# rlvc/FEALESS

Measured on AMD Instinct MI355X. Metric: frames/sec (640x480 RGB-D x N templates, 20 ICP iters), higher is better.
Workload: dtype u8

## Files before the change

### fealess_amd/csrc/fl_context.hip

```cpp
#include "fl_internal.h"
#include <stdlib.h>
#include <stdarg.h>
#include <string.h>
#include <algorithm>

int fl_set_error(fl_context *ctx, int code, const char *fmt, ...)
{
  if (ctx) {
    va_list ap;
    va_start(ap, fmt);
    vsnprintf(ctx->err, sizeof(ctx->err), fmt, ap);
    va_end(ap);
  }
  return code;
}

int fl_scratch(fl_context *ctx, size_t bytes, void **out)
{
  if (int rc = fl_context_join(ctx)) return rc;
  if (bytes > ctx->scratch_bytes) {
    if (ctx->scratch) {
      FL_HIP(ctx, hipStreamSynchronize(ctx->stream));
      FL_HIP(ctx, hipFree(ctx->scratch));
      ctx->scratch = nullptr;
// ... 59 lines not shown
  *out = ctx->icp_stream;
  return FL_OK;
}

extern "C" int fl_abi_version(void) { return FL_ABI_VERSION; }

struct FlOptionName { const char *name, *env; long fl_context::Options::*field; bool hex; long lo, hi; };
static const FlOptionName fl_option_names[] = {
  {"scan_prune", "FL_SCAN_PRUNE", &fl_context::Options::scan_prune, false, 0, 1},
  {"scan_prune_mid", "FL_SCAN_PRUNE_MID", &fl_context::Options::scan_prune_mid, true, -1, 0xFF},
  {"scan_prune_lanes", "FL_SCAN_PRUNE_LANES", &fl_context::Options::scan_prune_lanes, false, 0, 1},
  {"scan_prune_step", "FL_SCAN_PRUNE_STEP", &fl_context::Options::scan_prune_step, false, 0, 8},
  {"scan_first", "FL_SCAN_FIRST", &fl_context::Options::scan_first, false, 0, 16},
  {"icp_wide", "FL_ICP_WIDE", &fl_context::Options::icp_wide, false, -1, 1},
  {"icp_occ", "FL_ICP_OCC", &fl_context::Options::icp_occ, false, 0, 5},
  {"icp_order", "FL_ICP_ORDER", &fl_context::Options::icp_order, false, 0, 1},
  {"icp_wg_per_cu", "FL_ICP_WG_PER_CU", &fl_context::Options::icp_wg_per_cu, false, 0, 3},
  {"eager_frontend", "FL_EAGER_FRONTEND", &fl_context::Options::eager_frontend, false, 0, 1},
  {"dev_poison", "FL_DEV_POISON", &fl_context::Options::dev_poison, false, 0, 1},
  {"ws_pad", "FL_DEV_WS_PAD", &fl_context::Options::ws_pad, false, 0, 16l << 20},
  {"pipeline_icp", "FL_PIPELINE_ICP", &fl_context::Options::pipeline_icp, false, 0, 3},
  {"frontend_chunk_rows", "FL_FRONTEND_CHUNK_ROWS", &fl_context::Options::frontend_chunk_rows, false, 0, 60 * 1024},
  {"scan_run", "FL_SCAN_RUN", &fl_context::Options::scan_run, false, 0, 64},
  {"refine_lds", "FL_REFINE_LDS", &fl_context::Options::refine_lds, false, 0, 2},
  {"refine_lds_bytes", "FL_REFINE_LDS_BYTES", &fl_context::Options::refine_lds_bytes, false, 0, FL_REFINE_LDS_BYTES},
  {"verify_fused", "FL_VERIFY_FUSED", &fl_context::Options::verify_fused, false, 0, 1},
  {"verify_fused_px", "FL_VERIFY_FUSED_PX", &fl_context::Options::verify_fused_px, false, 0, FL_VERIFY_FUSED_PX},
};

static bool fl_option_valid(const FlOptionName &o, long v)
// ... 636 lines not shown
```

### fealess_amd/csrc/fl_icp.hip

```cpp
#include "fl_internal.h"
#include <float.h>
#include <math.h>
#include <string.h>
#include <type_traits>
#include <mutex>
#include <map>
#include <utility>

#define ICP_BS_SMALL 256
#define ICP_BS_WIDE 1024
#define ICP_DT 512
#ifdef FL_ICP_PHASES
#define TSTAMP(k) do { if (threadIdx.x == 0) { long long now_ = clock64(); S.tacc[k] += now_ - S.tlast; S.tlast = now_; } } while (0)
#define CH_STAMP_BEGIN long long c_add = 0, c_bar = 0, c_last = clock64()
#define CH_STAMP(v) { const long long now_ = clock64(); v += now_ - c_last; c_last = now_; }
#define CH_STAMP_END(k) { if (threadIdx.x == 0) { S.hist[k] += (unsigned)(c_add >> 4); S.hist[(k) + 1] += (unsigned)(c_bar >> 4); } }
#define PR_STAMP_BARRIER(k, every) { const long long b0_ = clock64(); tile_barrier(); if (threadIdx.x == 64) S.hist[k] += (unsigned)(((clock64() - b0_) * (every)) >> 4); }
#define ST_STAMP_BEGIN long long st_acc[6] = {0, 0, 0, 0, 0, 0}, st_last = clock64()
#define ST_STAMP(k) { const long long now_ = clock64(); st_acc[k] += now_ - st_last; st_last = now_; }
#define ST_ARRIVED(a, b) asm volatile("" :: "v"(a), "v"(b));
#define ST_STAMP_END { if ((threadIdx.x & 63) == 0) for (int k = 0; k < 5; ++k) atomicAdd(&S.stime[k], (unsigned long long)st_acc[k]); }
#else
#define TSTAMP(k) do { } while (0)
#define CH_STAMP_BEGIN
// ... 409 lines not shown
      const float v[8] = {c0.x, c0.y, c0.z, c0.w, c1.x, c1.y, c1.z, c1.w};
#pragma unroll
      for (int k = 0; k < 8; ++k) blk_term(bs, (k < 4 ? 4 * lane + k : 256 + 4 * lane + k - 4) < cnt ? v[k] : 0.0f, isum, bad);
      if (blk_finish(bs, isum, bad, acc)) continue;
    }
    float *dst = buf[b & 1];
    *(float4 *)(dst + 4 * lane) = c0;
    *(float4 *)(dst + 256 + 4 * lane) = c1;
    wave_lds_handover();
    if (lane == 0) acc = chain_tile<NBUF>(dst, cnt, acc);
    acc = uniform_f(acc);
  }
  return acc;
}

template <int MODE, bool DEFER, class SH>
__device__ __forceinline__ float l2dist_phase(SH &S, float *mod, const float *ref, bnd_t *bnd, float *dterm, int n, float thr,
                                             const float *Ropt, const float *Topt)
{
  constexpr bool parity = MODE == FL_ICP_PARITY && !DEFER;
  constexpr int TQ = parity ? SH::TQ : SH::BS;
  const int slot = parity ? S.producer_slot() : (int)threadIdx.x;
  const int clane = parity ? S.chain_lane() : -1;
  int counter = 0, inl = 0;
  double dsum[1] = {0.0};
  float acc = 0.0f;
  const int ntiles = (n + TQ - 1) / TQ;
  constexpr int KB = parity && !SH::BSUM ? ICP_BMACRO : 1;
  static_assert(KB == 1 || sizeof(S.prod) >= (size_t)2 * KB * TQ * sizeof(float), "two blocks of KB tiles of terms fit the A2 tiles");
  auto dbuf = [&](int t) -> float * {
    if (KB == 1) return S.dtile[t & 1];
    const int m = (t + KB - 1) / KB, first = m == 0 ? 0 : (m - 1) * KB + 1;
    return (float *)&S.prod[0][0][0] + ((m & 1) * KB + (t - first)) * TQ;
  };
  struct Row { F3 a, b; float bnd; };
  auto row_load = [&](Row &w, int t) {
    const int i = min(t * TQ + slot, n - 1);
    w.a = ld3_u32(mod, i);
    w.b = ld3_u32(ref, i);
    w.bnd = Ropt ? bnd_ld(bnd, i) : 0.0f;
  };
  auto row_process = [&](const Row &w, int t) {
    const int i = t * TQ + slot;
    float term = 0.0f;
    float a[3] = {w.a.x, w.a.y, w.a.z};
    const float b0 = w.b.x, b1 = w.b.y, b2 = w.b.z;
    if (i < n) {
      if (Ropt) {
        float move = 0.0f;
        if (vvalid(a[2])) {
          float o[3];
          mat_vec(Ropt, a, o);
          o[0] += Topt[0];
          o[1] += Topt[1];
          o[2] += Topt[2];
          const float mx = o[0] - a[0], my = o[1] - a[1], mz = o[2] - a[2];
          move = sqrt_upper(mx * mx + my * my + mz * mz);
          a[0] = o[0];
          a[1] = o[1];
          a[2] = o[2];
          mod[3 * i] = a[0];
// ... 163 lines not shown
__device__ __forceinline__ void pose_accumulate(SH &S)
{
  float RT[3];
  mat_vec(S.Ropt, S.T, RT);
  for (int k = 0; k < 3; ++k) S.T[k] = RT[k] + S.Topt[k];
  mat_mat(S.Ropt, S.R, S.R);
}
__device__ __forceinline__ void icp_result_none(fl_icp_result *res)
{
  for (int i = 0; i < 9; ++i) res->R[i] = 0.f;
  for (int i = 0; i < 3; ++i) res->T[i] = 0.f;
  res->dist_mean = -1.0f; res->px_ratio = 0.f;
  res->iters = 0; res->n_corr_last = 0;
}

template <int MODE, bool ORG, class SH>
__device__ __forceinline__ void icp_run(SH &S, uint8_t *wsb, const IcpWsLayout &L, int n_ref, int n_model,
                        int it_thr, float dmt, float ddt, fl_icp_result *res, const OrgGeom &og)
{
  constexpr int BS = SH::BS, NW = SH::NW;
  float *ref = (float *)(wsb + L.ref), *mod = (float *)(wsb + L.mod);
  float4 *sref = (float4 *)(wsb + L.sref);
  const float *jsrc = ORG ? (const float *)sref : ref;
  const int *idximg = ORG ? (const int *)((const uint8_t *)sref + org_idximg_offset(og.cw * og.ch)) : nullptr;
  int *nn = (int *)(wsb + L.nn);
  bnd_t *bnd = (bnd_t *)(wsb + L.bnd);
  float *nd = (float *)(wsb + L.nd), *dterm = (float *)(wsb + L.dterm);
  const int *perm = (const int *)(wsb + L.perm);
  const float *nrm = (const float *)(wsb + L.nrm);
  int *cell_start = (int *)(wsb + L.cell_start), *cell_cur = (int *)(wsb + L.cell_cur);
  constexpr bool plane = MODE == FL_ICP_POINT_TO_PLANE;
  constexpr int NSUM = plane ? 27 : 15;

  if (threadIdx.x == 0) {
    for (int i = 0; i < 9; ++i) S.R[i] = 0.f;
    for (int i = 0; i < 3; ++i) S.T[i] = 0.f;
    S.iter = 0;
    S.n_corr = 0;
    S.px = 0.f;
#ifdef FL_ICP_PHASES
    for (int i = 0; i < 16; ++i) S.tacc[i] = 0;
    for (int i = 0; i < 40; ++i) S.hist[i] = 0;
    for (int i = 0; i < 8; ++i) S.stime[i] = 0;
// ... 5 lines not shown
  if (n_model < 3 || n_ref < 3 || n_ref < n_model) {
    if (threadIdx.x == 0) icp_result_none(res);
    __syncthreads();
    return;
  }
  if (!ORG) build_grid(S, ref, n_ref, sref, cell_start, cell_cur, L.ncell_max);
  TSTAMP(0);
  for (int i = threadIdx.x; i < n_model; i += BS)
    if (!vvalid(mod[3 * i + 2])) { mod[3 * i] = 0.f; mod[3 * i + 1] = 0.f; mod[3 * i + 2] = 0.f; }
  if (threadIdx.x == 0) {
    S.R[0] = S.R[4] = S.R[8] = 1.f;
    S.dist_diff = FLT_MAX;
  }
  __syncthreads();
  constexpr bool SPEC = BS >= ICP_BS_WIDE && MODE == FL_ICP_PARITY && ORG;
  float mean_ub = l2dist_phase<MODE, SPEC>(S, mod, ref, bnd, dterm, n_model, FLT_MAX, nullptr, nullptr);
  int pending = SPEC ? 1 : 0;
  bool have_nn = false;
  float old_mean = 0.0f;

  const OrgSearchCtx ctx = org_search_ctx(mod, bnd, perm, (const float *)sref, (const float *)(wsb + L.zimg), n_model, og);
  auto chain_and_search = [&](const int pend, const bool want, const float r_lim, const float old_mean_) {
    if (pend && threadIdx.x < 64) {
      const float acc = chain_deferred<SH::CHAIN_NBUF>(dterm, S.dchain, n_model);
      if (threadIdx.x == 0) {
        const int counter = S.cnt, inl = S.inl;
        float dm = acc;
        if (counter > 0) dm /= (float)inl;
        const float new_mean = counter > 0 ? dm : FLT_MAX;
        S.px = counter > 0 ? (float)inl / (float)counter : 0.0f;
        if (pend == 2) {
          S.dist_diff = old_mean_ - new_mean;
          pose_accumulate(S);
        }
        S.dist_mean = new_mean;
        const bool go = (new_mean > dmt) && (S.dist_diff > ddt) && (S.iter < it_thr);
        *(volatile int *)&S.stop = go ? 0 : 1;
      }
    }
    if (want)
      org_search<SH, SPEC>(S, ctx, r_lim, true, [&](bool active, int i, float, float, float, int j, float d) {
        if (active) {
          nn[i] = j;
          nd[i] = d;
          if (j >= 0) bnd_st(bnd, i, sqrt_upper(d));
        }
      });
  };

  for (;;) {
    if (SPEC) {
      const int it_done = __builtin_amdgcn_readfirstlane(S.iter);
      const bool want = !have_nn && it_done >= 1 && it_done < it_thr;
      if (pending || want) {
        const float r_lim = pending ? sqrtf(3.0f * mean_ub) * 1.00001f : sqrtf(3 * S.dist_mean);
        if (threadIdx.x == 0) { S.a1_next = 0; S.stop = 0; }
        __syncthreads();
        chain_and_search(pending, want, uniform_f(r_lim), old_mean);
// ... 33 lines not shown
      } else if (!parity) {
        const float m[3] = {m0, m1, m2}, r[3] = {r0, r1, r2};
#pragma unroll
        for (int a = 0; a < 3; ++a)
#pragma unroll
          for (int b = 0; b < 3; ++b) ds[a * 3 + b] += (double)m[a] * (double)r[b];
#pragma unroll
        for (int q = 0; q < 3; ++q) { ds[9 + q] += (double)m[q]; ds[12 + q] += (double)r[q]; }
      }
    };
    if (!index_pairs && !SPEC) {
      const float r_thr = uniform_f(sqrtf(thr));
      auto on_found = [&](bool active, int i, float qx, float qy, float qz, int j, float d) {
        const bool keep = d <= thr;
        if (active) {
          nn[i] = keep ? j : -1;
          if (j >= 0) bnd_st(bnd, i, sqrt_upper(d));
        }
        if (keep) {
          ++kept;
          if (!parity) { const F3 rv = ld3_u32(jsrc, j); pair_sums(qx, qy, qz, rv.x, rv.y, rv.z, j); }
        }
      };
      if (ORG) {
        if (MODE == FL_ICP_PARITY && NW < 8) org_search_pipe(S, ctx, r_thr, on_found);
        else org_search<SH, SPEC>(S, ctx, r_thr, false, on_found);
      } else {
        const NnGrid G = nn_grid(S);
        int i = threadIdx.x;
        float qx = 0.f, qy = 0.f, qz = 0.f, qb = 0.f;
        if (i < n_model) { const F3 q3 = ld3_u32(mod, i); qx = q3.x; qy = q3.y; qz = q3.z; qb = bnd_ld(bnd, i); }
// ... 24 lines not shown
        bool in;
        F3 m, r;
      };
      constexpr bool ZIMG = ORG && NW < 8;
      const float *zimg = (const float *)(wsb + L.zimg);
      const float inv_cw = uniform_f(1.0f / (float)max(og.cw, 1));
      auto row_load = [&](Row &w, int t) {
        const int i = t * TQ + slot;
        w.in = i < rows;
        const int ic = min(i, rows - 1);
        w.j = ld_u32(nn, ic);
        w.d = SPEC ? ld_u32(nd, ic) : 0.0f;
        w.m = ld3_u32(mod, ic);
      };
      auto row_gather = [&](Row &w) {
        if (!(w.in && (!SPEC || w.d <= thr))) w.j = -1;
        if (ZIMG) w.r.x = ld_u32(zimg, max(w.j, 0));
        else w.r = ld3_u32(jsrc, max(w.j, 0));
      };
      auto row_write = [&](const Row &w, int t) {
        const bool have = w.j >= 0;
        if (SPEC && have) ++kept;
        float (*tile)[SH::TS] = S.prod[t & 1];
        F3 rp = w.r;
        if (ZIMG) {
          const int jj = max(w.j, 0);
          int vv, uu;
          if (ctx.small_crop) {
            vv = (int)(((float)jj + 0.5f) * inv_cw);
            uu = jj - __mul24(vv, og.cw);
            if (uu < 0) { --vv; uu += og.cw; } else if (uu >= og.cw) { ++vv; uu -= og.cw; }
// ... 47 lines not shown
    } else
    for (int t = 0; t < ntiles; ++t) {
      if (slot >= 0) {
        const int i = t * TQ + slot;
        float m[3] = {0.f, 0.f, 0.f}, r[3] = {0.f, 0.f, 0.f};
        bool have_m = false, have_pair = false;
        if (i < rows) {
          if (iter == 1) {
            if (i < n_model) {
              have_m = true;
              have_pair = true;
              if (vvalid(mod[3 * i + 2])) { m[0] = mod[3 * i]; m[1] = mod[3 * i + 1]; m[2] = mod[3 * i + 2]; }
            }
            if (vvalid(ref[3 * i + 2])) { r[0] = ref[3 * i]; r[1] = ref[3 * i + 1]; r[2] = ref[3 * i + 2]; }
          } else {
            const int j = nn[i];
            if (j >= 0) {
              have_m = have_pair = true;
              m[0] = mod[3 * i]; m[1] = mod[3 * i + 1]; m[2] = mod[3 * i + 2];
              r[0] = jsrc[3 * j]; r[1] = jsrc[3 * j + 1]; r[2] = jsrc[3 * j + 2];
            }
          }
        }
        if (parity) {
          float (*tile)[SH::TS] = S.prod[t & 1];
#pragma unroll
          for (int a = 0; a < 3; ++a)
#pragma unroll
            for (int b = 0; b < 3; ++b) tile[a * 3 + b][slot] = have_pair ? m[a] * r[b] : 0.0f;
#pragma unroll
          for (int q = 0; q < 3; ++q) { tile[9 + q][slot] = have_m ? m[q] : 0.0f; tile[12 + q][slot] = r[q]; }
// ... 31 lines not shown
      for (int k = 0; k < NSUM; ++k) dd[k] = (double)ds[k];
      block_sum_double<NSUM>(S, dd);
    }
    if (threadIdx.x == 0) {
      if (plane) solve_point_to_plane(S);
      else solve_rigid<MODE>(S, ncm, ncr);
    }
    __syncthreads();
    TSTAMP(4);
    if (!S.ok) continue;
    float Ro[9], To[3];
    for (int k = 0; k < 9; ++k) Ro[k] = S.Ropt[k];
    for (int k = 0; k < 3; ++k) To[k] = S.Topt[k];
    old_mean = S.dist_mean;
    __syncthreads();
    mean_ub = l2dist_phase<MODE, SPEC>(S, mod, ref, bnd, dterm, n_model, 3 * old_mean, Ro, To);
    TSTAMP(5);
    if (SPEC) {
      pending = 2;
      have_nn = false;
      continue;
    }
    if (threadIdx.x == 0) {
      S.dist_diff = old_mean - S.dist_mean;
      pose_accumulate(S);
    }
    __syncthreads();
  }
  if (threadIdx.x == 0) {
    for (int i = 0; i < 9; ++i) res->R[i] = S.R[i];
    for (int i = 0; i < 3; ++i) res->T[i] = S.T[i];
// ... 31 lines not shown
      su += (float)du * z;
      sv += (float)dv * z;
    }
  if (!ok) return;
  const float s2 = (float)((2 * ICP_NRM_R + 1) * ICP_NRM_R * (ICP_NRM_R + 1) * (2 * ICP_NRM_R + 1) / 3);
  const float zu = su / s2, zv = sv / s2, X = (x - cx) / fx, Y = (y - cy) / fy;
  const float pu[3] = {zc / fx + X * zu, Y * zu, zu}, pv[3] = {X * zv, zc / fy + Y * zv, zv};
  const float c[3] = {pu[1] * pv[2] - pu[2] * pv[1], pu[2] * pv[0] - pu[0] * pv[2], pu[0] * pv[1] - pu[1] * pv[0]};
  const float len = sqrtf(c[0] * c[0] + c[1] * c[1] + c[2] * c[2]);
  if (!(len > 0.f)) return;
  n[0] = c[0] / len; n[1] = c[1] / len; n[2] = c[2] / len;
}

template <class SH>
__device__ __forceinline__ int crop_clouds(SH &S, const IcpArgs &a, const uint16_t *scene, const uint16_t *model, bool model_01mm,
                           const int *rm, const int *rr, float *ref, float *mod, float *nrm, float *rimg, int *idximg, float *zimg)
{
  constexpr int BS = SH::BS, NW = SH::NW;
  const int cw = rm[2], ch = rm[3], np = cw * ch;
  const float inv_fx = 1.0f / a.fx, inv_fy = 1.0f / a.fy;
  const float minv_fx = 1.0f / 608.f, minv_fy = 1.0f / 608.f;
  const float zs = (float)(1 / 1000.0);
  const int lane = threadIdx.x & 63, wv = threadIdx.x >> 6;
  const float inv_cw = 1.0f / (float)cw;
  int kept_before = 0, step = 0;
  __syncthreads();
  for (int base = 0; base < np; base += BS, ++step) {
    const int p = base + threadIdx.x;
    float A[3] = {0, 0, 0}, B[3] = {0, 0, 0};
    float zsf_keep = NAN;
    int keep = 0;
// ... 23 lines not shown
    if (lane == 0) slot[wv] = __popcll(bal);
    __syncthreads();
    int before = 0, total = 0;
#pragma unroll
    for (int i = 0; i < NW; ++i) { const int c = slot[i]; before += i < wv ? c : 0; total += c; }
    if (p < np) {
      const F3 pt = {keep ? A[0] : INFINITY, keep ? A[1] : INFINITY, keep ? A[2] : INFINITY};
      __builtin_memcpy(rimg + 3 * p, &pt, 12);
      idximg[p] = keep ? kept_before + before + in_wave : NN_IDX_NONE;
      if (zimg) zimg[p] = keep ? zsf_keep : NAN;
    }
    if (keep) {
      const int k = kept_before + before + in_wave;
      ref[3 * k] = A[0]; ref[3 * k + 1] = A[1]; ref[3 * k + 2] = A[2];
      mod[3 * k] = B[0]; mod[3 * k + 1] = B[1]; mod[3 * k + 2] = B[2];
      if (nrm) {
        float nv[3];
        scene_normal(scene, a.w, a.h, rr[0] + p % cw, rr[1] + p / cw, a.fx, a.fy, a.cx, a.cy, nv);
        nrm[3 * k] = nv[0]; nrm[3 * k + 1] = nv[1]; nrm[3 * k + 2] = nv[2];
      }
    }
    kept_before += total;
  }
  if (threadIdx.x < 3 * NN_OVERRUN) rimg[3 * np + threadIdx.x] = INFINITY;
  if (zimg && threadIdx.x < NN_OVERRUN + 1) zimg[np + threadIdx.x] = NAN;
  __syncthreads();
  return kept_before;
}

template <class SH>
__device__ __forceinline__ void build_tile_order(SH &S, const int *idximg, int cw, int ch, int n, int *perm)
{
  constexpr int BS = SH::BS, NW = SH::NW;
  int *cnt = (int *)&S.prod[0][0][0];
  constexpr int CAP = (int)(sizeof(S.prod) / 4);
  constexpr int TW = ICP_TILE_W, TH = 64 / ICP_TILE_W;
  static_assert(TW * TH == 64 && (TW & (TW - 1)) == 0, "a tile is one wavefront of pixels");
  const int ntx = (cw + TW - 1) / TW, nty = (ch + TH - 1) / TH, ntile = ntx * nty;
  if (ntile > CAP) {
    for (int i = threadIdx.x; i < n; i += BS) perm[i] = i;
    __syncthreads();
    return;
  }
  const int lane = threadIdx.x & 63, wv = threadIdx.x >> 6;
  const float inv_ntx = 1.0f / (float)ntx;
  auto tile_index = [&](int t, bool &has) {
    const int ty = (int)(((float)t + 0.5f) * inv_ntx);
    int tx = t - ty * ntx;
    if (ty & 1) tx = ntx - 1 - tx;
    const int c = lane / TH, x = tx * TW + ((ty & 1) ? TW - 1 - c : c), y = ty * TH + (lane & (TH - 1));
    int k = NN_IDX_NONE;
    if (x < cw && y < ch) k = idximg[y * cw + x];
    has = (unsigned)k < (unsigned)NN_IDX_NONE;
    return k;
  };
// ... 15 lines not shown
      if (lane >= d) inc += v;
    }
    if (lane == 63) S.iscan[wv] = inc;
    __syncthreads();
    int before = 0;
#pragma unroll
    for (int w = 0; w < NW; ++w) before += w < wv ? S.iscan[w] : 0;
    int ex = before + inc - mine;
    for (int t = lo; t < hi; ++t) { const int c = cnt[t]; cnt[t] = ex; ex += c; }
  }
  __syncthreads();
  for (int t = wv; t < ntile; t += NW) {
    bool has;
    const int k = tile_index(t, has);
    const unsigned long long bal = __ballot(has);
    if (has) perm[cnt[t] + __builtin_amdgcn_mbcnt_hi((unsigned)(bal >> 32), __builtin_amdgcn_mbcnt_lo((unsigned)bal, 0u))] = k;
  }
  __syncthreads();
}

#define ICP_WPE(MODE, BS) ((BS) == ICP_BS_SMALL ? ICP_MODE_WPE(MODE) : (BS) / 256)

template <int MODE, int BS>
__global__ __launch_bounds__(BS) void k_icp_clouds(IcpArgs a)
{
  extern __shared__ __align__(16) uint8_t icp_smem[];
  using SH = IcpSharedT<BS>;
  SH &S = *(SH *)icp_smem;
  const IcpWsLayout L = icp_layout(a.n_max);
  uint8_t *wsb = a.ws + (size_t)blockIdx.x * a.ws_stride;
  const OrgGeom none = {};
  if (threadIdx.x == 0) S.cw = 0;
  __syncthreads();
  icp_run<MODE, false>(S, wsb, L, a.job.n_ref, a.job.n_model, a.it_thr, a.dmt, a.ddt, &a.results[blockIdx.x].det.icp, none);
}

template <int MODE, int BS, int WPE = ICP_WPE(MODE, BS)>
__global__ __launch_bounds__(BS) __attribute__((amdgpu_waves_per_eu(WPE, WPE > 4 ? WPE : 4)))
void k_icp_pipeline(IcpArgs a)
{
  extern __shared__ __align__(16) uint8_t icp_smem[];
  using SH = IcpSharedT<BS>;
  SH &S = *(SH *)icp_smem;
#ifdef FL_ICP_PHASES
  if (threadIdx.x == 0) { S.tkernel = clock64(); S.wall0 = wall_clock64(); }
#endif
  const int job = a.order ? a.order[blockIdx.x] : (int)blockIdx.x, rank = a.job.kind == 0 && !a.jobs ? job % a.ranks : 0;
  const int frame = a.job.kind == 0 ? (a.jobs ? a.jobs[job].frame : job / a.ranks) : job;
  const IcpWsLayout L = icp_layout(a.n_max);
  uint8_t *wsb = a.ws + (size_t)job * a.ws_stride;
  float *ref = (float *)(wsb + L.ref), *mod = (float *)(wsb + L.mod);

// ... 53 lines not shown
    const int *rm = S.rect_m, *rr = S.rect_r;
    const bool bad = rm[0] < 0 || rm[1] < 0 || rm[2] < 0 || rm[3] < 0 || rm[0] + rm[2] > a.w || rm[1] + rm[3] > a.h ||
                     rr[0] < 0 || rr[1] < 0 || rr[2] < 0 || rr[3] < 0 || rr[0] + rr[2] > a.w || rr[1] + rr[3] > a.h ||
                     rm[2] != rr[2] || rm[3] != rr[3] || (long long)rm[2] * rm[3] > a.n_max;
    if (bad) {
      if (threadIdx.x == 0) { res->status = FL_ERR_ASSERT; res->det.status = FL_ERR_ASSERT; res->found = 0; }
      return;
    }
  }
  if (threadIdx.x == 0) S.cw = 0;
  __syncthreads();
  float *rimg = (float *)(wsb + L.sref);
  const int np = crop_clouds(S, a, scene, model, model_01mm, S.rect_m, S.rect_r, ref, mod,
                             MODE == FL_ICP_POINT_TO_PLANE ? (float *)(wsb + L.nrm) : nullptr, rimg,
                             (int *)((uint8_t *)rimg + org_idximg_offset(S.rect_m[2] * S.rect_m[3])),
                             MODE == FL_ICP_PARITY && BS < ICP_BS_WIDE ? (float *)(wsb + L.zimg) : nullptr);
  const OrgGeom og = {__builtin_amdgcn_readfirstlane(S.rect_r[2]), __builtin_amdgcn_readfirstlane(S.rect_r[3]),
                      uniform_f((float)S.rect_r[0] - a.cx), uniform_f((float)S.rect_r[1] - a.cy), a.fx, a.fy,
                      __builtin_amdgcn_readfirstlane(S.rect_r[0]), __builtin_amdgcn_readfirstlane(S.rect_r[1]), a.cx, a.cy,
                      uniform_f(1.0f / a.fx), uniform_f(1.0f / a.fy)};
  build_tile_order(S, (const int *)((const uint8_t *)rimg + org_idximg_offset(og.cw * og.ch)), og.cw, og.ch, np, (int *)(wsb + L.perm));
  float mc[3] = {0, 0, 0}, rc[3] = {0, 0, 0};
  if (MODE == FL_ICP_PARITY) {
    {
      constexpr int TQ = SH::TQ;
      const int slot = S.producer_slot(), clane = S.chain_lane(), ntiles = (np + TQ - 1) / TQ;
      float acc = 0.0f;
      for (int t = 0; t < ntiles; ++t) {
        if (slot >= 0) {
          const int i = t * TQ + slot;
          F3 m3 = {0.f, 0.f, 0.f}, r3 = {0.f, 0.f, 0.f};
          if (i < np) { m3 = ld3_u32(mod, i); r3 = ld3_u32(ref, i); }
          float (*tile)[SH::TS] = S.prod[t & 1];
          tile[0][slot] = m3.x; tile[1][slot] = m3.y; tile[2][slot] = m3.z;
          tile[3][slot] = r3.x; tile[4][slot] = r3.y; tile[5][slot] = r3.z;
        } else if (t > 0 && clane >= 0 && clane < 6) {
// ... 18 lines not shown
      for (int k = 0; k < 3; ++k) { mc[k] = (float)(S.dsum[0][k] / np); rc[k] = (float)(S.dsum[0][3 + k] / np); }
  }
  float t_tmp[3], t_init[3];
  for (int k = 0; k < 3; ++k) { t_tmp[k] = rc[k] - mc[k]; t_init[k] = t_tmp[k] + t_match[k]; }
  __syncthreads();
  for (int i = threadIdx.x; i < np; i += BS) {
    if (!vvalid(mod[3 * i + 2])) continue;
    const float I[9] = {1, 0, 0, 0, 1, 0, 0, 0, 1};
    float v[3] = {mod[3 * i], mod[3 * i + 1], mod[3 * i + 2]}, o[3];
    mat_vec(I, v, o);
    mod[3 * i] = o[0] + t_tmp[0];
    mod[3 * i + 1] = o[1] + t_tmp[1];
    mod[3 * i + 2] = o[2] + t_tmp[2];
  }
  __syncthreads();
  icp_run<MODE, true>(S, wsb, L, np, np, a.it_thr, a.dmt, a.ddt, &res->det.icp, og);
  if (threadIdx.x == 0) {
    const fl_icp_result &ic = res->det.icp;
    float Rt[3];
    mat_vec(ic.R, t_init, Rt);
    for (int k = 0; k < 3; ++k) res->det.T_final[k] = Rt[k] + ic.T[k];
    mat_mat(ic.R, r_match, res->det.R_final);
    res->det.n_points = np;
    res->det.status = FL_OK;
    for (int i = 0; i < 3; ++i) {
      for (int j = 0; j < 3; ++j) res->pose[i * 4 + j] = res->det.R_final[i * 3 + j];
      res->pose[i * 4 + 3] = res->det.T_final[i];
    }
    res->pose[12] = res->pose[13] = res->pose[14] = 0.f;
    res->pose[15] = 1.f;
    res->found = 1;
// ... 138 lines not shown
  return FL_OK;
}
static bool icp_wide(fl_context *ctx, int n_jobs)
{
  if (ctx->opt.icp_wide == 0) return false;
  if (ctx->opt.icp_wide == 1) return true;
  return n_jobs <= 2 * ctx->cus;
}
static int icp_small_wpe(fl_context *ctx, int n_jobs)
{
  if (ctx->opt.icp_occ == 4 || ctx->opt.icp_occ == 5) return (int)ctx->opt.icp_occ;
  const int cus = ctx->cus;
  const int r4 = (n_jobs + 4 * cus - 1) / (4 * cus), r5 = (n_jobs + 5 * cus - 1) / (5 * cus);
  return 1.25 * r5 < 1.0 * r4 ? 5 : 4;
}
template <int MODE>
static int icp_launch_mode(fl_context *ctx, int n_jobs, const IcpArgs &a)
{
  const bool wide = icp_wide(ctx, n_jobs);
  if constexpr (MODE == FL_ICP_PARITY) {
    if (a.job.kind != 2 && !wide && icp_small_wpe(ctx, n_jobs) == 5)
      return icp_launch_one<ICP_BS_SMALL>(ctx, k_icp_pipeline<MODE, ICP_BS_SMALL, 5>, n_jobs, a);
  }
  if (a.job.kind == 2)
    return wide ? icp_launch_one<ICP_BS_WIDE>(ctx, k_icp_clouds<MODE, ICP_BS_WIDE>, n_jobs, a)
                : icp_launch_one<ICP_BS_SMALL>(ctx, k_icp_clouds<MODE, ICP_BS_SMALL>, n_jobs, a);
  return wide ? icp_launch_one<ICP_BS_WIDE>(ctx, k_icp_pipeline<MODE, ICP_BS_WIDE>, n_jobs, a)
              : icp_launch_one<ICP_BS_SMALL>(ctx, k_icp_pipeline<MODE, ICP_BS_SMALL>, n_jobs, a);
}
static int icp_launch(fl_context *ctx, int n_jobs, const IcpArgs &a)
{
  switch (a.mode) {
    case FL_ICP_PARITY: return icp_launch_mode<FL_ICP_PARITY>(ctx, n_jobs, a);
    case FL_ICP_FAST: return icp_launch_mode<FL_ICP_FAST>(ctx, n_jobs, a);
    case FL_ICP_POINT_TO_PLANE: return icp_launch_mode<FL_ICP_POINT_TO_PLANE>(ctx, n_jobs, a);
    default: return fl_set_error(ctx, FL_ERR_INVALID, "unknown fl_icp_mode");
  }
// ... 233 lines not shown
```

### fealess_amd/csrc/fl_icp_search.h

```cpp
#pragma once

template <typename T>
__device__ __forceinline__ T ld_u32(const T *__restrict__ base, int idx)
{
  return *(const T *)((const char *)base + (size_t)((unsigned)idx * (unsigned)sizeof(T)));
}

struct F3 { float x, y, z; };
__device__ __forceinline__ F3 ld3_u32(const float *__restrict__ base, int i)
{
  F3 v;
  unsigned i3;
  asm("v_lshl_add_u32 %0, %1, 1, %1" : "=v"(i3) : "v"(i));
  __builtin_memcpy(&v, (const char *)base + (size_t)(i3 << 2), 12);
  return v;
}

typedef uint16_t bnd_t;
__host__ __device__ __forceinline__ uint16_t bnd_pack(unsigned bits)
{
  return (uint16_t)(((bits < 0x7FC00000u ? bits : 0x7FC00000u) + 0xFFFFu) >> 16);
}
__device__ __forceinline__ float bnd_ld(const bnd_t *__restrict__ b, int i) { return __uint_as_float((unsigned)ld_u32(b, i) << 16); }
__device__ __forceinline__ void bnd_st(bnd_t *b, int i, float v) { b[i] = bnd_pack(__float_as_uint(v)); }
// ... 313 lines not shown
  if (isfinite(r) && zlo > 1.0f) {
    const float ilo = __builtin_amdgcn_rcpf(zlo), ihi = __builtin_amdgcn_rcpf(zhi);
    const float xlo = qx - r, xhi = qx + r, ylo = qy - r, yhi = qy + r;
    const int iul = cvt_i32_sat(ceilf((xlo * (xlo < 0.f ? ilo : ihi)) * g.fx - cul));
    const int iuh = cvt_i32_sat(floorf((xhi * (xhi > 0.f ? ilo : ihi)) * g.fx - cuh));
    const int ivl = cvt_i32_sat(ceilf((ylo * (ylo < 0.f ? ilo : ihi)) * g.fy - cvl));
    const int ivh = cvt_i32_sat(floorf((yhi * (yhi > 0.f ? ilo : ihi)) * g.fy - cvh));
    u_lo = max(iul, 0);
    u_hi = min(iuh, g.cw - 1);
    v_lo = max(ivl, 0);
    v_hi = min(ivh, g.ch - 1);
  }
  return u_lo <= u_hi && v_lo <= v_hi;
}

struct OrgSearchCtx {
  const float *mod;
  const bnd_t *bnd;
  const int *perm;
  const float *rimg, *zimg;
  int n_model;
  OrgGeom og;
  int last_s, last_pt;
  float cwf;
  bool small_crop;
};
__device__ __forceinline__ OrgSearchCtx org_search_ctx(const float *mod, const bnd_t *bnd, const int *perm, const float *rimg, const float *zimg,
                                                       int n_model, const OrgGeom &og)
{
  return {mod, bnd, perm, rimg, zimg, n_model, og, n_model - 1, og.cw * og.ch + NN_OVERRUN - 1, (float)og.cw,
          (long long)og.cw * og.ch + NN_OVERRUN < (1 << 24)};
}
template <class SH>
__device__ __forceinline__ float4 *org_stage(SH &S, int wv)
{
  static_assert(sizeof(S.prod) + sizeof(S.dtile) + sizeof(S.stage_pad) >= (size_t)SH::NW * ICP_STAGE_CAP * 16, "the chain tiles (idle during the search) hold every wave's staged rows");
  static_assert(offsetof(SH, stage_pad) == offsetof(SH, dtile) + sizeof(S.dtile) && offsetof(SH, dtile) == offsetof(SH, prod) + sizeof(S.prod),
                "prod, dtile and stage_pad are one contiguous region");
  return (float4 *)&S.prod[0][0][0] + wv * ICP_STAGE_CAP;
}
__device__ __forceinline__ float4 org_image_point(const OrgSearchCtx &c, int pos)
{
  const F3 pt = ld3_u32(c.rimg, pos);
  return nn_point(pt.x, pt.y, pt.z, pt.x == INFINITY ? NN_IDX_NONE : pos);
}

__device__ __forceinline__ unsigned long long org_scan(const OrgSearchCtx &c, float qx, float qy, float qz, int u_lo, int u_hi, int v_lo, int v_hi,
                                                       int maxw, int maxh)
{
  constexpr int NBQ = ICP_NBQ;
  unsigned long long best = NN_KEY_NONE;
  const int wl = u_hi - u_lo, hl = v_hi - v_lo, RS = c.og.cw;
  const int b0 = v_lo * RS + u_lo;
  static_assert(NBQ - 1 <= NN_OVERRUN, "the overrun guard behind the image is NN_OVERRUN points");
  const int wlc = max(wl - (NBQ - 1), 0);
  for (int dv = 0; dv < maxh; ++dv) {
    const int rb = b0 + min(dv, hl) * RS;
    for (int du = 0; du < maxw; du += NBQ) {
      float4 cur[NBQ];
      const int bb = rb + min(du, wlc);
#pragma unroll
      for (int e = 0; e < NBQ; ++e) cur[e] = org_image_point(c, bb + e);
// ... 26 lines not shown
  const int wlc = max(wl - 3, 0);
  for (int dv = 0; dv < maxh; ++dv) {
    const float4 *rowp = row0 + __mul24(min(dv, hl), W);
    for (int du = 0; du < 4 * nbw; du += 4) {
      const float4 *bp = rowp + min(du, wlc);
      float4 cur[4];
#pragma unroll
      for (int e = 0; e < 4; ++e) cur[e] = bp[e];
#pragma unroll
      for (int e = 0; e < 4; ++e) NN_CONSIDER(cur[e])
    }
  }
  return best;
}

template <class SH, bool SPEC, class F>
__device__ __forceinline__ void org_search(SH &S, const OrgSearchCtx &c, const float r_lim, const bool poll_stop, F &&found)
{
  const OrgGeom &og = c.og;
  const int n_model = c.n_model;
  const int lane = threadIdx.x & 63, wv = __builtin_amdgcn_readfirstlane((int)threadIdx.x >> 6);
  float4 *stage = org_stage(S, wv);
  const float cul = uniform_f(og.offu + 0.01f), cuh = uniform_f(og.offu - 0.01f), cvl = uniform_f(og.offv + 0.01f), cvh = uniform_f(og.offv - 0.01f);
  constexpr int stride = SH::NW * 64;
  int static_next = wv * 64 + 4 * stride;
  auto claim = [&](int count) {
    int v = 0;
    if (lane == 0) v = atomicAdd(&S.a1_next, count);
    return __builtin_amdgcn_readfirstlane(v);
  };
  auto next_step = [&]() {
    if (SPEC) return claim(64);
// ... 108 lines not shown
  return r;
}
struct Prep {
  int i;
  float qx, qy, qz;
  bool active, queryable;
  int u_lo, u_hi, v_lo, v_hi;
  int U0, V0, W, maxh, nbw, npass;
  bool w3;
#ifdef FL_ICP_PHASES
  int wlmax;
#endif
  bool any, staged;
  float z[ICP_PIPE_NP];
};
template <class SH, class F>
__device__ __forceinline__ void org_search_pipe(SH &S, const OrgSearchCtx &c, const float r_lim, F &&found)
{
  const OrgGeom &og = c.og;
  const int n_model = c.n_model, last_pt = c.last_pt;
  const int lane = threadIdx.x & 63, wv = __builtin_amdgcn_readfirstlane((int)threadIdx.x >> 6);
  float4 *stage = org_stage(S, wv);
  const float lanef = (float)lane;
  const float cul = uniform_f(og.offu + 0.01f), cuh = uniform_f(og.offu - 0.01f), cvl = uniform_f(og.offv + 0.01f), cvh = uniform_f(og.offv - 0.01f);
  constexpr int stride = SH::NW * 64;
  auto prepare = [&](Prep &P, int sb, int i, const F3 &q, float b) {
    P.i = i; P.qx = q.x; P.qy = q.y; P.qz = q.z;
    P.active = sb + lane < n_model;
    P.queryable = P.active && r_lim >= 0.f && isfinite(q.x) && isfinite(q.y) && isfinite(q.z);
    int u_lo, u_hi, v_lo, v_hi;
    const bool some = org_window2_flat(og, cul, cuh, cvl, cvh, q.x, q.y, q.z, nn_radius(q.x, q.y, q.z, fminf(b, r_lim)), P.queryable,
                                       u_lo, u_hi, v_lo, v_hi);
// ... 108 lines not shown
```

### fealess_amd/csrc/fl_internal.h

```cpp
#pragma once
#include <hip/hip_runtime.h>
#include <cmath>
#include <stdint.h>
#include <stdio.h>
#include <string>
#include <vector>
#include "../../include/fealess_hip.h"

#define FL_WAVE 64

struct fl_context {
  int device = 0;
  hipStream_t own_stream = nullptr;
  hipStream_t stream = nullptr;
  hipStream_t icp_stream = nullptr;
  long icp_stream_mode = 0;
  hipEvent_t ev_icp_tail = nullptr;
  bool icp_pending = false;
  char err[512] = {0};
  void *scratch = nullptr;
  size_t scratch_bytes = 0;
  void *pinned = nullptr;
  size_t pinned_bytes = 0;
  int cus = 256;
  struct Options {
    long scan_prune = 1;
    long scan_prune_mid = -1;
    long scan_prune_lanes = 1;
    long scan_prune_step = 0;
    long scan_first = 0;
    long icp_wide = -1;
    long icp_occ = 0;
    long icp_order = 1;
    long icp_wg_per_cu = 0;
    long eager_frontend = 0;
    long dev_poison = 0;
    long ws_pad = 0;
    long pipeline_icp = 3;
    long frontend_chunk_rows = 0;
    long scan_run = 0;
    long refine_lds = 0;
    long refine_lds_bytes = 0;
    long verify_fused = 0;
    long verify_fused_px = 0;
  } opt;
  bool verify_fused_attr = false;
  int detectors = 0;
// ... 406 lines not shown
```

Before: 90330.

## Use 16-bit NN/perm indices and pixel-index ref reconstruction in small parity ICP

Adds an IDX template parameter so the 256-thread parity organised-search ICP kernel can store nearest-neighbour and tile-permutation indices as uint16 when the crop has at most 65535 points. It also stores a 16-bit pixel index plus reference depth per kept point and rebuilds the reference point from the image geometry in the L2 distance phase, instead of loading three floats. Both changes aim to cut global memory traffic per ICP iteration, at the cost of extra integer/float arithmetic and reuse of the dterm/nd workspace slots. The option defaults to -1, which counts as enabled.

After: 92470 (median of 6 runs). +2.4%, better.

```diff
diff --git a/fealess_amd/csrc/fl_context.hip b/fealess_amd/csrc/fl_context.hip
--- a/fealess_amd/csrc/fl_context.hip
+++ b/fealess_amd/csrc/fl_context.hip
@@ -97,6 +97,7 @@
   {"scan_first", "FL_SCAN_FIRST", &fl_context::Options::scan_first, false, 0, 16},
   {"icp_wide", "FL_ICP_WIDE", &fl_context::Options::icp_wide, false, -1, 1},
   {"icp_occ", "FL_ICP_OCC", &fl_context::Options::icp_occ, false, 0, 5},
+  {"icp_idx16", "FL_ICP_IDX16", &fl_context::Options::icp_idx16, false, -1, 1},
   {"icp_order", "FL_ICP_ORDER", &fl_context::Options::icp_order, false, 0, 1},
   {"icp_wg_per_cu", "FL_ICP_WG_PER_CU", &fl_context::Options::icp_wg_per_cu, false, 0, 3},
   {"eager_frontend", "FL_EAGER_FRONTEND", &fl_context::Options::eager_frontend, false, 0, 1},
diff --git a/fealess_amd/csrc/fl_icp.hip b/fealess_amd/csrc/fl_icp.hip
--- a/fealess_amd/csrc/fl_icp.hip
+++ b/fealess_amd/csrc/fl_icp.hip
@@ -447,9 +447,9 @@
   return acc;
 }
 
-template <int MODE, bool DEFER, class SH>
+template <int MODE, bool DEFER, bool REFPIX, class SH>
 __device__ __forceinline__ float l2dist_phase(SH &S, float *mod, const float *ref, bnd_t *bnd, float *dterm, int n, float thr,
-                                             const float *Ropt, const float *Topt)
+                                             const float *Ropt, const float *Topt, const uint16_t *pix, const float *zref, const OrgGeom &og)
 {
   constexpr bool parity = MODE == FL_ICP_PARITY && !DEFER;
   constexpr int TQ = parity ? SH::TQ : SH::BS;
@@ -466,18 +466,26 @@
     const int m = (t + KB - 1) / KB, first = m == 0 ? 0 : (m - 1) * KB + 1;
     return (float *)&S.prod[0][0][0] + ((m & 1) * KB + (t - first)) * TQ;
   };
-  struct Row { F3 a, b; float bnd; };
+  struct Row { F3 a, b; float bnd; int p; };
+  const float inv_cw = REFPIX ? uniform_f(1.0f / (float)max(og.cw, 1)) : 0.0f;
   auto row_load = [&](Row &w, int t) {
     const int i = min(t * TQ + slot, n - 1);
     w.a = ld3_u32(mod, i);
-    w.b = ld3_u32(ref, i);
+    if (REFPIX) { w.p = ld_u32(pix, i); w.b.x = ld_u32(zref, i); }
+    else w.b = ld3_u32(ref, i);
     w.bnd = Ropt ? bnd_ld(bnd, i) : 0.0f;
   };
   auto row_process = [&](const Row &w, int t) {
     const int i = t * TQ + slot;
     float term = 0.0f;
     float a[3] = {w.a.x, w.a.y, w.a.z};
-    const float b0 = w.b.x, b1 = w.b.y, b2 = w.b.z;
+    F3 rp = w.b;
+    if (REFPIX) {
+      int vv = (int)(((float)w.p + 0.5f) * inv_cw), uu = w.p - __mul24(vv, og.cw);
+      if (uu < 0) { --vv; uu += og.cw; } else if (uu >= og.cw) { ++vv; uu -= og.cw; }
+      rp = org_point(og, uu, vv, w.b.x);
+    }
+    const float b0 = rp.x, b1 = rp.y, b2 = rp.z;
     if (i < n) {
       if (Ropt) {
         float move = 0.0f;
@@ -671,7 +679,9 @@
   res->iters = 0; res->n_corr_last = 0;
 }
 
-template <int MODE, bool ORG, class SH>
+template <class IDX>
+__device__ __forceinline__ int nn_get(IDX v) { return sizeof(IDX) == 2 && (int)v == 0xFFFF ? -1 : (int)v; }
+template <int MODE, bool ORG, class IDX, class SH>
 __device__ __forceinline__ void icp_run(SH &S, uint8_t *wsb, const IcpWsLayout &L, int n_ref, int n_model,
                         int it_thr, float dmt, float ddt, fl_icp_result *res, const OrgGeom &og)
 {
@@ -680,10 +690,14 @@
   float4 *sref = (float4 *)(wsb + L.sref);
   const float *jsrc = ORG ? (const float *)sref : ref;
   const int *idximg = ORG ? (const int *)((const uint8_t *)sref + org_idximg_offset(og.cw * og.ch)) : nullptr;
-  int *nn = (int *)(wsb + L.nn);
+  constexpr bool IDX16 = sizeof(IDX) == 2;
+  static_assert(!IDX16 || (MODE == FL_ICP_PARITY && ORG && SH::NW < 8), "16-bit indices: the 256-thread parity kernel of the organised search only");
+  IDX *nn = (IDX *)(wsb + L.nn);
   bnd_t *bnd = (bnd_t *)(wsb + L.bnd);
   float *nd = (float *)(wsb + L.nd), *dterm = (float *)(wsb + L.dterm);
-  const int *perm = (const int *)(wsb + L.perm);
+  const IDX *perm = (const IDX *)(wsb + L.perm);
+  const uint16_t *pix = (const uint16_t *)(wsb + L.dterm);
+  const float *zref = (const float *)(wsb + L.nd);
   const float *nrm = (const float *)(wsb + L.nrm);
   int *cell_start = (int *)(wsb + L.cell_start), *cell_cur = (int *)(wsb + L.cell_cur);
   constexpr bool plane = MODE == FL_ICP_POINT_TO_PLANE;
@@ -719,12 +733,13 @@
   }
   __syncthreads();
   constexpr bool SPEC = BS >= ICP_BS_WIDE && MODE == FL_ICP_PARITY && ORG;
-  float mean_ub = l2dist_phase<MODE, SPEC>(S, mod, ref, bnd, dterm, n_model, FLT_MAX, nullptr, nullptr);
+  static_assert(!(IDX16 && SPEC), "pix[] / zref[] live where the deferred chain keeps dterm[] / nd[]");
+  float mean_ub = l2dist_phase<MODE, SPEC, false>(S, mod, ref, bnd, dterm, n_model, FLT_MAX, nullptr, nullptr, pix, zref, og);
   int pending = SPEC ? 1 : 0;
   bool have_nn = false;
   float old_mean = 0.0f;
 
-  const OrgSearchCtx ctx = org_search_ctx(mod, bnd, perm, (const float *)sref, (const float *)(wsb + L.zimg), n_model, og);
+  const auto ctx = org_search_ctx(mod, bnd, perm, (const float *)sref, (const float *)(wsb + L.zimg), n_model, og);
   auto chain_and_search = [&](const int pend, const bool want, const float r_lim, const float old_mean_) {
     if (pend && threadIdx.x < 64) {
       const float acc = chain_deferred<SH::CHAIN_NBUF>(dterm, S.dchain, n_model);
@@ -746,7 +761,7 @@
     if (want)
       org_search<SH, SPEC>(S, ctx, r_lim, true, [&](bool active, int i, float, float, float, int j, float d) {
         if (active) {
-          nn[i] = j;
+          nn[i] = (IDX)j;
           nd[i] = d;
           if (j >= 0) bnd_st(bnd, i, sqrt_upper(d));
         }
@@ -810,7 +825,7 @@
       auto on_found = [&](bool active, int i, float qx, float qy, float qz, int j, float d) {
         const bool keep = d <= thr;
         if (active) {
-          nn[i] = keep ? j : -1;
+          nn[i] = (IDX)(keep ? j : -1);
           if (j >= 0) bnd_st(bnd, i, sqrt_upper(d));
         }
         if (keep) {
@@ -865,7 +880,7 @@
         w.m = ld3_u32(mod, ic);
       };
       auto row_gather = [&](Row &w) {
-        if (!(w.in && (!SPEC || w.d <= thr))) w.j = -1;
+        if (!(w.in && (!SPEC || w.d <= thr)) || (IDX16 && w.j == 0xFFFF)) w.j = -1;
         if (ZIMG) w.r.x = ld_u32(zimg, max(w.j, 0));
         else w.r = ld3_u32(jsrc, max(w.j, 0));
       };
@@ -943,7 +958,7 @@
             }
             if (vvalid(ref[3 * i + 2])) { r[0] = ref[3 * i]; r[1] = ref[3 * i + 1]; r[2] = ref[3 * i + 2]; }
           } else {
-            const int j = nn[i];
+            const int j = nn_get(nn[i]);
             if (j >= 0) {
               have_m = have_pair = true;
               m[0] = mod[3 * i]; m[1] = mod[3 * i + 1]; m[2] = mod[3 * i + 2];
@@ -1005,7 +1020,7 @@
     for (int k = 0; k < 3; ++k) To[k] = S.Topt[k];
     old_mean = S.dist_mean;
     __syncthreads();
-    mean_ub = l2dist_phase<MODE, SPEC>(S, mod, ref, bnd, dterm, n_model, 3 * old_mean, Ro, To);
+    mean_ub = l2dist_phase<MODE, SPEC, IDX16>(S, mod, ref, bnd, dterm, n_model, 3 * old_mean, Ro, To, pix, zref, og);
     TSTAMP(5);
     if (SPEC) {
       pending = 2;
@@ -1067,7 +1082,8 @@
 
 template <class SH>
 __device__ __forceinline__ int crop_clouds(SH &S, const IcpArgs &a, const uint16_t *scene, const uint16_t *model, bool model_01mm,
-                           const int *rm, const int *rr, float *ref, float *mod, float *nrm, float *rimg, int *idximg, float *zimg)
+                           const int *rm, const int *rr, float *ref, float *mod, float *nrm, float *rimg, int *idximg, float *zimg,
+                           uint16_t *pix, float *zref)
 {
   constexpr int BS = SH::BS, NW = SH::NW;
   const int cw = rm[2], ch = rm[3], np = cw * ch;
@@ -1121,6 +1137,7 @@
       const int k = kept_before + before + in_wave;
       ref[3 * k] = A[0]; ref[3 * k + 1] = A[1]; ref[3 * k + 2] = A[2];
       mod[3 * k] = B[0]; mod[3 * k + 1] = B[1]; mod[3 * k + 2] = B[2];
+      if (pix) { pix[k] = (uint16_t)p; zref[k] = zsf_keep; }
       if (nrm) {
         float nv[3];
         scene_normal(scene, a.w, a.h, rr[0] + p % cw, rr[1] + p / cw, a.fx, a.fy, a.cx, a.cy, nv);
@@ -1135,8 +1152,8 @@
   return kept_before;
 }
 
-template <class SH>
-__device__ __forceinline__ void build_tile_order(SH &S, const int *idximg, int cw, int ch, int n, int *perm)
+template <class SH, class IDX>
+__device__ __forceinline__ void build_tile_order(SH &S, const int *idximg, int cw, int ch, int n, IDX *perm)
 {
   constexpr int BS = SH::BS, NW = SH::NW;
   int *cnt = (int *)&S.prod[0][0][0];
@@ -1145,7 +1162,15 @@
   static_assert(TW * TH == 64 && (TW & (TW - 1)) == 0, "a tile is one wavefront of pixels");
   const int ntx = (cw + TW - 1) / TW, nty = (ch + TH - 1) / TH, ntile = ntx * nty;
   if (ntile > CAP) {
-    for (int i = threadIdx.x; i < n; i += BS) perm[i] = i;
+    if constexpr (sizeof(IDX) == 2) {
+      for (unsigned i = threadIdx.x; i < (unsigned)n; i += BS) {
+        unsigned o = 2 * i;
+        asm volatile("" : "+v"(o));
+        *(IDX *)((char *)perm + (size_t)o) = (IDX)i;
+      }
+    } else {
+      for (int i = threadIdx.x; i < n; i += BS) perm[i] = i;
+    }
     __syncthreads();
     return;
   }
@@ -1191,7 +1216,7 @@
     bool has;
     const int k = tile_index(t, has);
     const unsigned long long bal = __ballot(has);
-    if (has) perm[cnt[t] + __builtin_amdgcn_mbcnt_hi((unsigned)(bal >> 32), __builtin_amdgcn_mbcnt_lo((unsigned)bal, 0u))] = k;
+    if (has) perm[cnt[t] + __builtin_amdgcn_mbcnt_hi((unsigned)(bal >> 32), __builtin_amdgcn_mbcnt_lo((unsigned)bal, 0u))] = (IDX)k;
   }
   __syncthreads();
 }
@@ -1209,10 +1234,10 @@
   const OrgGeom none = {};
   if (threadIdx.x == 0) S.cw = 0;
   __syncthreads();
-  icp_run<MODE, false>(S, wsb, L, a.job.n_ref, a.job.n_model, a.it_thr, a.dmt, a.ddt, &a.results[blockIdx.x].det.icp, none);
-}
-
-template <int MODE, int BS, int WPE = ICP_WPE(MODE, BS)>
+  icp_run<MODE, false, int>(S, wsb, L, a.job.n_ref, a.job.n_model, a.it_thr, a.dmt, a.ddt, &a.results[blockIdx.x].det.icp, none);
+}
+
+template <int MODE, int BS, int WPE = ICP_WPE(MODE, BS), class IDX = int>
 __global__ __launch_bounds__(BS) __attribute__((amdgpu_waves_per_eu(WPE, WPE > 4 ? WPE : 4)))
 void k_icp_pipeline(IcpArgs a)
 {
@@ -1296,12 +1321,13 @@
   const int np = crop_clouds(S, a, scene, model, model_01mm, S.rect_m, S.rect_r, ref, mod,
                              MODE == FL_ICP_POINT_TO_PLANE ? (float *)(wsb + L.nrm) : nullptr, rimg,
                              (int *)((uint8_t *)rimg + org_idximg_offset(S.rect_m[2] * S.rect_m[3])),
-                             MODE == FL_ICP_PARITY && BS < ICP_BS_WIDE ? (float *)(wsb + L.zimg) : nullptr);
+                             MODE == FL_ICP_PARITY && BS < ICP_BS_WIDE ? (float *)(wsb + L.zimg) : nullptr,
+                             sizeof(IDX) == 2 ? (uint16_t *)(wsb + L.dterm) : nullptr, (float *)(wsb + L.nd));
   const OrgGeom og = {__builtin_amdgcn_readfirstlane(S.rect_r[2]), __builtin_amdgcn_readfirstlane(S.rect_r[3]),
                       uniform_f((float)S.rect_r[0] - a.cx), uniform_f((float)S.rect_r[1] - a.cy), a.fx, a.fy,
                       __builtin_amdgcn_readfirstlane(S.rect_r[0]), __builtin_amdgcn_readfirstlane(S.rect_r[1]), a.cx, a.cy,
                       uniform_f(1.0f / a.fx), uniform_f(1.0f / a.fy)};
-  build_tile_order(S, (const int *)((const uint8_t *)rimg + org_idximg_offset(og.cw * og.ch)), og.cw, og.ch, np, (int *)(wsb + L.perm));
+  build_tile_order(S, (const int *)((const uint8_t *)rimg + org_idximg_offset(og.cw * og.ch)), og.cw, og.ch, np, (IDX *)(wsb + L.perm));
   float mc[3] = {0, 0, 0}, rc[3] = {0, 0, 0};
   if (MODE == FL_ICP_PARITY) {
     {
@@ -1350,7 +1376,7 @@
     mod[3 * i + 2] = o[2] + t_tmp[2];
   }
   __syncthreads();
-  icp_run<MODE, true>(S, wsb, L, np, np, a.it_thr, a.dmt, a.ddt, &res->det.icp, og);
+  icp_run<MODE, true, IDX>(S, wsb, L, np, np, a.it_thr, a.dmt, a.ddt, &res->det.icp, og);
   if (threadIdx.x == 0) {
     const fl_icp_result &ic = res->det.icp;
     float Rt[3];
@@ -1519,13 +1545,22 @@
   const int r4 = (n_jobs + 4 * cus - 1) / (4 * cus), r5 = (n_jobs + 5 * cus - 1) / (5 * cus);
   return 1.25 * r5 < 1.0 * r4 ? 5 : 4;
 }
+static bool icp_idx16(fl_context *ctx, const IcpArgs &a)
+{
+  return ctx->opt.icp_idx16 != 0 && a.n_max <= 65535;
+}
 template <int MODE>
 static int icp_launch_mode(fl_context *ctx, int n_jobs, const IcpArgs &a)
 {
   const bool wide = icp_wide(ctx, n_jobs);
   if constexpr (MODE == FL_ICP_PARITY) {
-    if (a.job.kind != 2 && !wide && icp_small_wpe(ctx, n_jobs) == 5)
-      return icp_launch_one<ICP_BS_SMALL>(ctx, k_icp_pipeline<MODE, ICP_BS_SMALL, 5>, n_jobs, a);
+    if (a.job.kind != 2 && !wide) {
+      const bool five = icp_small_wpe(ctx, n_jobs) == 5;
+      if (icp_idx16(ctx, a))
+        return five ? icp_launch_one<ICP_BS_SMALL>(ctx, k_icp_pipeline<MODE, ICP_BS_SMALL, 5, uint16_t>, n_jobs, a)
+                    : icp_launch_one<ICP_BS_SMALL>(ctx, k_icp_pipeline<MODE, ICP_BS_SMALL, ICP_PARITY_WPE, uint16_t>, n_jobs, a);
+      if (five) return icp_launch_one<ICP_BS_SMALL>(ctx, k_icp_pipeline<MODE, ICP_BS_SMALL, 5>, n_jobs, a);
+    }
   }
   if (a.job.kind == 2)
     return wide ? icp_launch_one<ICP_BS_WIDE>(ctx, k_icp_clouds<MODE, ICP_BS_WIDE>, n_jobs, a)
diff --git a/fealess_amd/csrc/fl_icp_search.h b/fealess_amd/csrc/fl_icp_search.h
--- a/fealess_amd/csrc/fl_icp_search.h
+++ b/fealess_amd/csrc/fl_icp_search.h
@@ -351,10 +351,11 @@
   return u_lo <= u_hi && v_lo <= v_hi;
 }
 
+template <class IDX>
 struct OrgSearchCtx {
   const float *mod;
   const bnd_t *bnd;
-  const int *perm;
+  const IDX *perm;
   const float *rimg, *zimg;
   int n_model;
   OrgGeom og;
@@ -362,8 +363,9 @@
   float cwf;
   bool small_crop;
 };
-__device__ __forceinline__ OrgSearchCtx org_search_ctx(const float *mod, const bnd_t *bnd, const int *perm, const float *rimg, const float *zimg,
-                                                       int n_model, const OrgGeom &og)
+template <class IDX>
+__device__ __forceinline__ OrgSearchCtx<IDX> org_search_ctx(const float *mod, const bnd_t *bnd, const IDX *perm, const float *rimg, const float *zimg,
+                                                            int n_model, const OrgGeom &og)
 {
   return {mod, bnd, perm, rimg, zimg, n_model, og, n_model - 1, og.cw * og.ch + NN_OVERRUN - 1, (float)og.cw,
           (long long)og.cw * og.ch + NN_OVERRUN < (1 << 24)};
@@ -376,13 +378,15 @@
                 "prod, dtile and stage_pad are one contiguous region");
   return (float4 *)&S.prod[0][0][0] + wv * ICP_STAGE_CAP;
 }
-__device__ __forceinline__ float4 org_image_point(const OrgSearchCtx &c, int pos)
+template <class IDX>
+__device__ __forceinline__ float4 org_image_point(const OrgSearchCtx<IDX> &c, int pos)
 {
   const F3 pt = ld3_u32(c.rimg, pos);
   return nn_point(pt.x, pt.y, pt.z, pt.x == INFINITY ? NN_IDX_NONE : pos);
 }
 
-__device__ __forceinline__ unsigned long long org_scan(const OrgSearchCtx &c, float qx, float qy, float qz, int u_lo, int u_hi, int v_lo, int v_hi,
+template <class IDX>
+__device__ __forceinline__ unsigned long long org_scan(const OrgSearchCtx<IDX> &c, float qx, float qy, float qz, int u_lo, int u_hi, int v_lo, int v_hi,
                                                        int maxw, int maxh)
 {
   constexpr int NBQ = ICP_NBQ;
@@ -439,8 +443,8 @@
   return best;
 }
 
-template <class SH, bool SPEC, class F>
-__device__ __forceinline__ void org_search(SH &S, const OrgSearchCtx &c, const float r_lim, const bool poll_stop, F &&found)
+template <class SH, bool SPEC, class IDX, class F>
+__device__ __forceinline__ void org_search(SH &S, const OrgSearchCtx<IDX> &c, const float r_lim, const bool poll_stop, F &&found)
 {
   const OrgGeom &og = c.og;
   const int n_model = c.n_model;
@@ -579,8 +583,8 @@
   bool any, staged;
   float z[ICP_PIPE_NP];
 };
-template <class SH, class F>
-__device__ __forceinline__ void org_search_pipe(SH &S, const OrgSearchCtx &c, const float r_lim, F &&found)
+template <class SH, class IDX, class F>
+__device__ __forceinline__ void org_search_pipe(SH &S, const OrgSearchCtx<IDX> &c, const float r_lim, F &&found)
 {
   const OrgGeom &og = c.og;
   const int n_model = c.n_model, last_pt = c.last_pt;
diff --git a/fealess_amd/csrc/fl_internal.h b/fealess_amd/csrc/fl_internal.h
--- a/fealess_amd/csrc/fl_internal.h
+++ b/fealess_amd/csrc/fl_internal.h
@@ -31,6 +31,7 @@
     long scan_first = 0;
     long icp_wide = -1;
     long icp_occ = 0;
+    long icp_idx16 = -1;
     long icp_order = 1;
     long icp_wg_per_cu = 0;
     long eager_frontend = 0;
```
